# maxim2266/csvplus

Measured on AMD Instinct MI355X. Metric: joined rows/sec (IndexOn build + chained Join, 1e8-row 3-col orders), higher is better.
Workload: dtype u32; 1 GPU; BASELINE configs[3]: orders(1e8 x {cust_id,prod_id,qty}).Join(UniqueIndexOn customers.id 1e7).Join(UniqueIndexOn products.prod_id 1e5); rows=100000000, customers=10000000, products=100000, rows_this_rank=100000000, exchange=none (1 GPU), output=sorted positions

## Files before the change

csvplus_amd/csrc/chain.hip:

```cpp
#include <type_traits>

#include "probe_device.hpp"

namespace cph {

constexpr int kChainThreads = 256;
constexpr int kChainWaves   = kChainThreads / kWave;
constexpr int kChainRows    = 8;
constexpr int kWaveTile     = kWave * kChainRows;
constexpr int kChainTile    = kChainThreads * kChainRows;
constexpr int kChainMasks   = kChainRows * kChainWaves;
constexpr int kMaxChain     = 4;

struct ChainStepArg {
    DevCol col;
    const uint8_t* codec;
    const uint32_t* rowtab;
    const uint2* ranktab;
    int32_t positions;
    int32_t ranktab_lds;
    const uint4* hash;
    uint32_t hash_sectors;
    uint32_t hash_slice_mask;
    int32_t src;
// ... 340 lines not shown
        uint32_t wave_matches = 0;
        const uint64_t mword = (tile * kChainWaves + wave) * kChainRows;
#pragma unroll
        for (int k = 0; k < kChainRows; k++) {
            const bool ok = (okm >> k) & 1u;
            const uint64_t bal = __ballot(ok);
            wave_matches += (uint32_t)__popcll(bal);
            if (lane == 0) masks[mword + k] = bal;
            if (ok) {
#pragma unroll
                for (int s = 0; s < S; s++) (a.out_rows[s] + wr.rbase)[wr.rel[k]] = brow[s][k];
            }
        }
        if (lane == 0) wave_counts[tile * kChainWaves + wave] = wave_matches;
    }
}

__global__ __launch_bounds__(256) void k_sum_counts(const uint32_t* __restrict__ counts, uint64_t n,
                                                   unsigned long long* __restrict__ total) {
    __shared__ uint64_t s_w[256 / kWave];
    uint64_t t = 0;
    const uint64_t stride = (uint64_t)gridDim.x * 256;
    for (uint64_t i = (uint64_t)blockIdx.x * 256 + threadIdx.x; i < n; i += stride) t += counts[i];
    t = wave_sum(t);
    if (lane_id() == 0) s_w[wave_id()] = t;
    __syncthreads();
    if (threadIdx.x == 0) {
        uint64_t r = 0;
        for (int w = 0; w < 256 / kWave; w++) r += s_w[w];
        if (r) atomicAdd(total, (unsigned long long)r);
    }
}

__global__ __launch_bounds__(256) void k_sum_counts_report(const uint32_t* __restrict__ counts, uint64_t n, unsigned long long* __restrict__ acc,
                                                          uint32_t* __restrict__ ticket, unsigned long long* __restrict__ host_out) {
    __shared__ uint64_t s_w[256 / kWave];
    uint64_t t = 0;
    const uint64_t stride = (uint64_t)gridDim.x * 256;
    for (uint64_t i = (uint64_t)blockIdx.x * 256 + threadIdx.x; i < n; i += stride) t += counts[i];
    t = wave_sum(t);
    if (lane_id() == 0) s_w[wave_id()] = t;
    __syncthreads();
    if (threadIdx.x == 0) {
        uint64_t r = 0;
        for (int w = 0; w < 256 / kWave; w++) r += s_w[w];
        if (r) atomicAdd(acc, (unsigned long long)r);
        __threadfence();
        if (atomicAdd(ticket, 1u) == gridDim.x - 1u) {
            const unsigned long long total = atomicExch(acc, 0ull);
            atomicExch(ticket, 0u);
            *host_out = total;
            __threadfence_system();
        }
    }
}

template <int S>
__global__ __launch_bounds__(kChainThreads) void k_chain_compact(ChainArgs dense_rows, uint64_t probe_base,
                                                                const uint64_t* __restrict__ masks,
                                                                const uint32_t* __restrict__ wave_base, uint64_t ntiles,
                                                                uint64_t* __restrict__ out_stream, ChainArgs out_rows) {
    const int lane = lane_id(), wave = wave_id();
    const uint64_t lt = lanemask_lt();
    for (uint64_t tile = blockIdx.x; tile < ntiles; tile += gridDim.x) {
        const uint64_t wt = tile * kChainWaves + wave;
        uint64_t pos = wave_base[wt];
#pragma unroll
        for (int k = 0; k < kChainRows; k++) {
            const uint64_t m = masks[wt * kChainRows + k];
            if ((m >> lane) & 1ull) {
                const uint64_t row = wt * kWaveTile + (uint64_t)k * kWave + lane;
                const uint64_t p = pos + (uint64_t)__popcll(m & lt);
                out_stream[p] = probe_base + row;
#pragma unroll
                for (int s = 0; s < S; s++) out_rows.out_rows[s][p] = dense_rows.out_rows[s][row];
            }
            pos += (uint64_t)__popcll(m);
        }
    }
}

__global__ void k_compose_u64(const uint64_t* __restrict__ src, const uint64_t* __restrict__ idx, uint64_t* __restrict__ dst,
                              uint64_t n) {
    const uint64_t stride = (uint64_t)gridDim.x * blockDim.x;
// ... 261 lines not shown
         {&k_chain_dense<S, false, true, false>, &k_chain_dense<S, false, true, true>}},
        {{&k_chain_dense<S, true, false, false>, &k_chain_dense<S, true, false, true>},
         {&k_chain_dense<S, true, true, false>, &k_chain_dense<S, true, true, true>}}};
    KernelFn kernel = variants[long_keys ? 1 : 0][wide ? 1 : 0][(dbg && !dep) ? 1 : 0];
    if (!dbg && ctx->chain_rows4 != 0 && ((S == 2 && long_keys && wide) || (S >= 3 && (long_keys || wide)) || S == 4 || ctx->chain_rows4 == 2)) {
        static const KernelFn r4[2][2] = {{&k_chain_dense<S, false, false, false, 0u, 4>, &k_chain_dense<S, false, true, false, 0u, 4>},
                                          {&k_chain_dense<S, true, false, false, 0u, 4>, &k_chain_dense<S, true, true, false, 0u, 4>}};
        kernel = r4[long_keys ? 1 : 0][wide ? 1 : 0];
    }
    if constexpr (S >= 2) {
        if (dep) kernel = &k_chain_dense<S, true, true, false, 0u, 4, true>;
    }
    if (lean) {
        constexpr uint32_t kAll = (1u << S) - 1u;
        if (lean == kAll) kernel = &k_chain_dense<S, false, false, false, kAll>;
        if constexpr (S == 2) {
            if (lean == 1u) kernel = &k_chain_dense<S, false, false, false, 1u>;
            if (lean == 2u) kernel = &k_chain_dense<S, false, false, false, 2u>;
        }
    }
    int per_cu = 1, cus = 256;
    CPH_TRY(kernel_setup(ctx, reinterpret_cast<const void*>(kernel), kChainThreads, lds, &per_cu));
    CPH_TRY(device_cus(ctx, &cus));
    const unsigned grid = (unsigned)std::min<uint64_t>(ntiles, (uint64_t)cus * (uint64_t)per_cu);
    {
        ProfScope ps(ctx, prof_name, 0);
        hipLaunchKernelGGL(kernel, dim3(grid), dim3(kChainThreads), lds, ctx->stream, args, nprobe, probe_base,
                           ntiles, d_masks, d_counts, dep ? 0 : dbg, largs);
    }
    if (host_total) {
        DevBuf& acc = ctx->self_clean[ctx->stream_slot].sum;
        CPH_TRY(self_clean_block(ctx, &acc, 16));
        ProfScope ps(ctx, "k_sum_counts", 4.0 * (double)ncounts);
        const unsigned sgrid = (unsigned)std::min<uint64_t>((ncounts + 255) / 256, 512);
        hipLaunchKernelGGL(k_sum_counts_report, dim3(sgrid), dim3(256), 0, ctx->stream, d_counts, ncounts, acc.as<unsigned long long>(),
                           acc.as<uint32_t>() + 2, reinterpret_cast<unsigned long long*>(host_total));
    } else if (d_total) {
        ProfScope ps(ctx, "k_sum_counts", 4.0 * (double)ncounts);
        CPH_HIP_TRY(hipMemsetAsync(d_total, 0, sizeof(uint64_t), ctx->stream));
        const unsigned sgrid = (unsigned)std::min<uint64_t>((ncounts + 255) / 256, 512);
        hipLaunchKernelGGL(k_sum_counts, dim3(sgrid), dim3(256), 0, ctx->stream, d_counts, ncounts,
                           reinterpret_cast<unsigned long long*>(d_total));
    }
    CPH_HIP_TRY(hipGetLastError());
    if (args_out) *args_out = args;
    if (grid_out) *grid_out = grid;
    return {};
}

bool chain_fast_path_ok(const ChainStep* steps, int nsteps);

Status chain_enqueue_dense(cph_ctx* ctx, const ChainStep* steps, int nsteps, uint64_t nprobe, uint64_t probe_base,
                           uint32_t* const* d_rows, uint64_t* d_masks, uint32_t* d_counts, uint64_t* d_total, bool positions) {
    switch (nsteps) {
    case 1: return enqueue_dense<1>(ctx, steps, nprobe, probe_base, d_rows, d_masks, d_counts, d_total, nullptr, nullptr, positions);
    case 2: return enqueue_dense<2>(ctx, steps, nprobe, probe_base, d_rows, d_masks, d_counts, d_total, nullptr, nullptr, positions);
    case 3: return enqueue_dense<3>(ctx, steps, nprobe, probe_base, d_rows, d_masks, d_counts, d_total, nullptr, nullptr, positions);
    case 4: return enqueue_dense<4>(ctx, steps, nprobe, probe_base, d_rows, d_masks, d_counts, d_total, nullptr, nullptr, positions);
    }
    return {CPH_ERR_INVALID, "bad chain length"};
}
template <int S>
static Status enqueue_codes(cph_ctx* ctx, const cph_index* const* idx, const uint32_t* const* d_codes, uint64_t nprobe, uint32_t* const* d_rows,
                            uint64_t* d_masks, uint32_t* d_counts, uint64_t* d_total, bool positions) {
    const uint64_t ntiles = (nprobe + kChainTile - 1) / kChainTile;
    CodeArgs args{};
    for (int s = 0; s < S; s++) {
        const cph_index* ix = idx[s];
        if (ix->nkeycols < 1 || ix->codec.nwords != 1 || !ix->codec.key32 || !ix->windows.empty() || ix->first_dup != UINT64_MAX)
// ... 83 lines not shown
    for (int s = 0; s < S; s++) {
        if (steps[s].source == 0) {
            ind[ni] = steps[s];
            irows[ni++] = rows[s];
            continue;
        }
        const int t = (steps[s].source < 0 ? -steps[s].source : steps[s].source) - 1;
        const int j = pa.n++;
        dep_of[s] = j;
        pa.src_dep[j] = dep_of[t];
        pa.src_rows[j] = rows[t];
        pa.tab[j] = tabs[s].as<uint32_t>();
        pa.out_rows[j] = rows[s];
    }
    switch (ni) {
    case 1: CPH_TRY(enqueue_dense<1>(ctx, ind, nprobe, probe_base, irows, masks, counts, nullptr, nullptr, grid_out, positions)); break;
    case 2: CPH_TRY(enqueue_dense<2>(ctx, ind, nprobe, probe_base, irows, masks, counts, nullptr, nullptr, grid_out, positions)); break;
    case 3: CPH_TRY(enqueue_dense<3>(ctx, ind, nprobe, probe_base, irows, masks, counts, nullptr, nullptr, grid_out, positions)); break;
    default: return {CPH_ERR_INVALID, "a chain needs a step keyed by the stream"};
    }
    {
        int per_cu = 1, cus = 256;
        CPH_TRY(kernel_setup(ctx, reinterpret_cast<const void*>(&k_chain_prejoined), kChainThreads, 0, &per_cu));
        CPH_TRY(device_cus(ctx, &cus));
        const unsigned grid = (unsigned)std::min<uint64_t>(ntiles, (uint64_t)cus * (uint64_t)per_cu);
        ProfScope ps(ctx, "k_chain_prejoined", (double)nprobe * 8.0 * pa.n);
        hipLaunchKernelGGL(k_chain_prejoined, dim3(grid), dim3(kChainThreads), 0, ctx->stream, pa, nprobe, ntiles, masks, counts);
        CPH_HIP_TRY(hipGetLastError());
    }
    {
        DevBuf& acc = ctx->self_clean[ctx->stream_slot].sum;
        CPH_TRY(self_clean_block(ctx, &acc, 16));
        ProfScope ps(ctx, "k_sum_counts", 4.0 * (double)ncounts);
        const unsigned sgrid = (unsigned)std::min<uint64_t>((ncounts + 255) / 256, 512);
        hipLaunchKernelGGL(k_sum_counts_report, dim3(sgrid), dim3(256), 0, ctx->stream, counts, ncounts, acc.as<unsigned long long>(),
                           acc.as<uint32_t>() + 2, reinterpret_cast<unsigned long long*>(host_total));
        CPH_HIP_TRY(hipGetLastError());
    }
    return {};
}

template <int S>
static Status run_fast(cph_ctx* ctx, const ChainStep* steps, uint64_t nprobe, uint64_t probe_base, ChainOut* out, bool positions) {
    const uint64_t ntiles = (nprobe + kChainTile - 1) / kChainTile;
    const uint64_t ncounts = ntiles * kChainWaves;
    uint32_t* rows[kMaxChain] = {nullptr};
    for (int s = 0; s < S; s++) {
        CPH_TRY(out->build_row[s].alloc(&ctx->pool, nprobe * sizeof(uint32_t)));
        rows[s] = out->build_row[s].as<uint32_t>();
    }
    DevBuf masks, counts;
    CPH_TRY(masks.alloc(&ctx->pool, ntiles * kChainMasks * sizeof(uint64_t)));
    CPH_TRY(counts.alloc(&ctx->pool, ncounts * sizeof(uint32_t)));
    volatile uint64_t* h = reinterpret_cast<volatile uint64_t*>(host_word(ctx, 2));
    if (!h) return {CPH_ERR_HIP, "no pinned host memory for the match total"};
    ChainArgs args{};
    unsigned grid = 1;
    bool prejoin = ctx->chain_prejoin != 0;
    {
        bool dep = false;
        for (int s = 0; s < S; s++) {
            if (steps[s].source == 0) continue;
            dep = true;
            const int t = (steps[s].source < 0 ? -steps[s].source : steps[s].source) - 1;
            if (steps[t].index->nrows * 2 > nprobe) prejoin = false;
        }
        prejoin = prejoin && dep;
    }
    if (prejoin) {
// ... 30 lines not shown
    for (int s = 0; s < S; s++) out->build_row[s] = std::move(fin.build_row[s]);
    return {};
}

static Status prejoin_general_step(cph_ctx* ctx, const ChainStep* steps, int s, int t, const uint32_t* h, const uint32_t* h_perm, uint64_t n_in, bool positions,
                                   DevBuf* cur_stream, DevBuf* cur_rows, uint64_t* n_out, bool* all) {
    const uint64_t nt = steps[s].cols[0].nrows;
    ChainStep one = steps[s];
    one.source = 0;
    DevBuf tab, tmask, tcount;
    CPH_TRY(tab.alloc(&ctx->pool, nt * sizeof(uint32_t)));
    CPH_TRY(tmask.alloc(&ctx->pool, chain_dense_mask_words(nt) * sizeof(uint64_t)));
    CPH_TRY(tcount.alloc(&ctx->pool, chain_dense_count_words(nt) * sizeof(uint32_t)));
    CPH_HIP_TRY(hipMemsetAsync(tab.get(), 0xFF, nt * sizeof(uint32_t), ctx->stream));
    uint32_t* r1[kMaxChain] = {tab.as<uint32_t>(), nullptr, nullptr, nullptr};
    CPH_TRY(enqueue_dense<1>(ctx, &one, nt, 0, r1, tmask.as<uint64_t>(), tcount.as<uint32_t>(), nullptr, nullptr, nullptr, positions, nullptr,
                             "k_chain_prejoin_table"));
    const uint64_t ntiles = (n_in + kPjTile - 1) / kPjTile;
    DevBuf v, counts;
    CPH_TRY(v.alloc(&ctx->pool, n_in * sizeof(uint32_t)));
    CPH_TRY(counts.alloc(&ctx->pool, (ntiles + 1) * sizeof(uint32_t)));
    volatile uint64_t* host_total = reinterpret_cast<volatile uint64_t*>(host_word(ctx, 2));
    if (!host_total) return {CPH_ERR_HIP, "no pinned host memory for the match total"};
    {
        ProfScope ps(ctx, "k_prejoin_tuples", (double)n_in * (h_perm ? 16.0 : 12.0));
        hipLaunchKernelGGL(k_prejoin_tuples, dim3((unsigned)ntiles), dim3(kPjThreads), 0, ctx->stream, tab.as<uint32_t>(), h, h_perm, n_in, v.as<uint32_t>(),
                           counts.as<uint32_t>());
        CPH_HIP_TRY(hipGetLastError());
    }
    {
        DevBuf& acc = ctx->self_clean[ctx->stream_slot].sum;
        CPH_TRY(self_clean_block(ctx, &acc, 16));
        ProfScope ps(ctx, "k_sum_counts", 4.0 * (double)ntiles);
        const unsigned sgrid = (unsigned)std::min<uint64_t>((ntiles + 255) / 256, 512);
        hipLaunchKernelGGL(k_sum_counts_report, dim3(sgrid), dim3(256), 0, ctx->stream, counts.as<uint32_t>(), ntiles, acc.as<unsigned long long>(),
                           acc.as<uint32_t>() + 2, reinterpret_cast<unsigned long long*>(const_cast<uint64_t*>(host_total)));
        CPH_HIP_TRY(hipGetLastError());
    }
    CPH_HIP_TRY(hipStreamSynchronize(ctx->stream));
    const uint64_t m = host_total[0];
    *all = m == n_in;
    *n_out = m;
    if (m == n_in) {
        cur_rows[s] = std::move(v);
        return {};
    }
    if (m == 0) return {};
    CPH_TRY(exclusive_scan_u32(ctx, counts.as<uint32_t>(), ntiles));
    PjCompactArgs ca{};
    DevBuf nstream, nrows[CPH_MAX_CHAIN];
    CPH_TRY(nstream.alloc(&ctx->pool, m * sizeof(uint64_t)));
    ca.src64 = cur_stream->as<uint64_t>();
    ca.dst64 = nstream.as<uint64_t>();
    for (int u = 0; u < s; u++) {
        CPH_TRY(nrows[u].alloc(&ctx->pool, m * sizeof(uint32_t)));
        ca.src32[ca.n32] = cur_rows[u].as<uint32_t>();
        ca.dst32[ca.n32++] = nrows[u].as<uint32_t>();
    }
    CPH_TRY(nrows[s].alloc(&ctx->pool, m * sizeof(uint32_t)));
    ca.src32[ca.n32] = v.as<uint32_t>();
    ca.dst32[ca.n32++] = nrows[s].as<uint32_t>();
    {
        ProfScope ps(ctx, "k_compose", (double)n_in * (12.0 + 4.0 * s) + (double)m * (12.0 + 4.0 * s));
        hipLaunchKernelGGL(k_prejoin_compact, dim3((unsigned)ntiles), dim3(kPjThreads), 0, ctx->stream, ca, v.as<uint32_t>(), n_in, counts.as<uint32_t>());
        CPH_HIP_TRY(hipGetLastError());
    }
    *cur_stream = std::move(nstream);
    for (int u = 0; u <= s; u++) cur_rows[u] = std::move(nrows[u]);
    return {};
// ... 101 lines not shown
```

csvplus_amd/csrc/keycodec.hip:

```cpp
#include <algorithm>
#include <cmath>
#include <mutex>

#include "codec_device.hpp"
#include "host_encode_kernels.hpp"

namespace cph {

constexpr int kStatsThreads = 256;
constexpr int kStatsRows = 8;

template <class B, bool SEG>
__global__ __launch_bounds__(kStatsThreads) void k_col_stats(DevCol col, uint32_t* __restrict__ g_minmax,
                                                            uint32_t* __restrict__ g_mask) {
    __shared__ __attribute__((aligned(16))) uint8_t s_flag[kMaxKeyBytes * 256];
    __shared__ uint32_t s_min, s_max;
    {
        uint4* z = reinterpret_cast<uint4*>(s_flag);
        for (int i = threadIdx.x; i < kMaxKeyBytes * 256 / 16; i += kStatsThreads) z[i] = make_uint4(0, 0, 0, 0);
    }
    if (threadIdx.x == 0) { s_min = 0xFFFFFFFFu; s_max = 0; }
    __syncthreads();

    uint32_t mn = 0xFFFFFFFFu, mx = 0;
// ... 1015 lines not shown
                const bool ok = hit[k] && v[k].len <= vmax && plen[k] <= (uint32_t)kWideBytes && slen[k] <= smaxlen;
                if (!ok && base + (uint64_t)k * kSplitThreads + threadIdx.x < tile_end) missed = 1;
                acc[k] = (OUT)(hit[k] ? e[k] - 1 : 0u) * pmult;
                v[k].window(plen[k], &w0[k], &w1[k]);
            }
            for (uint32_t q = 0; q < smaxlen; q++) {
                const CPH_LDS OUT* lp = s_lutw + q * (uint32_t)kLutStride;
#pragma unroll
                for (int k = 0; k < kSplitRows; k++) {
                    const uint64_t src = q < 8u ? w0[k] : w1[k];
                    const uint32_t sym = q < slen[k] ? ((uint32_t)(src >> (8u * (q & 7u))) & 0xFFu) + 1u : 0u;
                    acc[k] += lp[sym];
                }
            }
#pragma unroll
            for (int k = 0; k < kSplitRows; k++) {
                const uint64_t i = base + (uint64_t)k * kSplitThreads + threadIdx.x;
                if (i < tile_end) {
                    if (inv && acc[k] >= inv) missed = 1;
                    out[i] = acc[k];
                    if (counts) atomicAdd(&s_hist[(uint32_t)acc[k] & digit_mask], 1u);
                }
            }
        }
        if (counts) {
            lds_atomics_barrier();
            for (uint32_t x = threadIdx.x; x < bins; x += kSplitThreads) counts[(uint64_t)x * ntiles + tile] = s_hist[x];
            __syncthreads();
        }
    }
    if (__ballot(missed) && lane_id() == 0) *miss = 1u;
}

__global__ __launch_bounds__(kSplitThreads) void k_sample_fixed8(DevCol col, uint64_t step, uint64_t n, SplitSample* __restrict__ out,
                                                                SplitSample* __restrict__ host_out) {
    __shared__ uint32_t s_mask[8 * 8];
    __shared__ uint32_t s_last;
    const uint32_t W = col.fixed_width;
    if (threadIdx.x < 64) s_mask[threadIdx.x] = 0;
    __syncthreads();
    const uint64_t stride = (uint64_t)gridDim.x * kSplitThreads;
    for (uint64_t i = (uint64_t)blockIdx.x * kSplitThreads + threadIdx.x; i < n; i += stride) {
        uint64_t b, l;
        value_span_whole(col, i * step, &b, &l);
        ValueRegs<1> v;
        v.load(col, b, l);
        for (uint32_t q = 0; q < W; q++) {
            const uint32_t byte = (uint32_t)(v.c[0] >> (8u * q)) & 0xFFu, bit = 1u << (byte & 31u);
            uint32_t* w = &s_mask[q * 8u + (byte >> 5)];
            if (!(*(volatile uint32_t*)w & bit)) atomicOr(w, bit);
        }
    }
    lds_atomics_barrier();
    if (threadIdx.x < 64) {
        const uint32_t bits = s_mask[threadIdx.x];
        uint32_t* gm = &out->mask[0][0] + threadIdx.x;
        if (bits && (__hip_atomic_load(gm, __ATOMIC_RELAXED, __HIP_MEMORY_SCOPE_AGENT) & bits) != bits) atomicOr(gm, bits);
    }
    uint32_t* ticket = reinterpret_cast<uint32_t*>(out + 1);
    __threadfence();
    __syncthreads();
    if (threadIdx.x == 0) s_last = atomicAdd(ticket, 1u) == gridDim.x - 1u ? 1u : 0u;
    __syncthreads();
    if (s_last) {
        uint32_t* src = &out->mask[0][0];
        uint32_t* dst = &host_out->mask[0][0];
        for (uint32_t i = threadIdx.x; i < (uint32_t)(kSplitMaxValue * 8); i += kSplitThreads) dst[i] = i < 64u ? atomicExch(&src[i], 0u) : 0u;
        if (threadIdx.x == 0) {
            host_out->maxlen = W;
            host_out->minlen_inv = ~W;
            atomicExch(ticket, 0u);
        }
        __threadfence_system();
    }
}

int codec_virtual_cols(const CodecHost& cd, const DevCol* real, int nreal, DevCol* out) {
    int nv = 0;
    for (int c = 0; c < nreal; c++) {
        if (cd.has_split() && c == cd.split_col) {
            DevCol a = real[c], b = real[c];
            a.split = b.split = (uint16_t)(0x100u | cd.split_byte);
            a.part = 0;
            b.part = 1;
            out[nv++] = a;
            out[nv++] = b;
        } else {
            out[nv++] = real[c];
        }
    }
    return nv;
}

bool codec_wide_perfect_hash(CodecHost* codec) {
    CodecHost& cd = *codec;
    const size_t n = cd.wdict.size();
    cd.wide_disp.clear();
    cd.wide_slots.clear();
    if (n == 0 || n > (size_t)kWideDictMax) return false;
    std::vector<uint32_t> h(n);
// ... 142 lines not shown
        for (int sym = 0; sym < kLutStride; sym++) trial.lut[((size_t)p0 + i) * kLutStride + (size_t)sym] = 0;
    }
    trial.split_col = c;
    trial.split_byte = (uint8_t)d;
    trial.split_maxlen = (int32_t)st.vmax;
    trial.wdict = std::move(dict);
    if (!codec_wide_perfect_hash(&trial)) return {};
    CPH_TRY(codec_split_words(&trial));
    if (ctx->codec_debug)
        fprintf(stderr, "codec_try_split: column %d cut at 0x%02x: %zu prefixes (<= %u bytes), suffix %u..%u bytes: %d word(s), %d bits, sort cost %.0f (plain: %.1f bits%s)\n",
                c, d, trial.wdict.size(), st.pmax, smin, st.smax, trial.nwords, trial.word_bits[0], codec_sort_cost(trial), plain_bits,
                stats ? "" : " by the sample");
    *out = std::move(trial);
    *usable = true;
    return {};
}

bool codec_sample_applies(const cph_ctx* ctx, const DevCol* cols, int32_t ncols, uint64_t n) {
    return ctx->stats_sample != 0 && ncols == 1 && cols[0].fixed_width >= 1 && cols[0].fixed_width <= (uint32_t)kSplitMaxValue &&
           !cols[0].segmented() && n >= (1ull << 20);
}
size_t codec_sample_bytes() { return sizeof(SplitSample); }
Status codec_sample_launch(cph_ctx* ctx, const DevCol& col, uint64_t n, const void** host_copy) {
    const uint64_t step = n >> 16;
    const uint64_t nsel = (n + step - 1) / step;
    DevBuf& acc = ctx->self_clean[ctx->stream_slot].sample;
    CPH_TRY(self_clean_block(ctx, &acc, sizeof(SplitSample) + 16));
    uint32_t* hw = host_word(ctx, (uint32_t)(sizeof(SplitSample) / 4));
    if (!hw) return {CPH_ERR_HIP, "no pinned host memory for the sample's statistics"};
    ProfScope ps(ctx, "k_split_count", 0);
    uint64_t nblk = (nsel + kSplitThreads - 1) / kSplitThreads;
    if (nblk > 1024) nblk = 1024;
    if (col.fixed_width <= 8)
        hipLaunchKernelGGL(k_sample_fixed8, dim3((unsigned)nblk), dim3(kSplitThreads), 0, ctx->stream, col, step, nsel, acc.as<SplitSample>(),
                           reinterpret_cast<SplitSample*>(hw));
    else
        hipLaunchKernelGGL(k_split_count, dim3((unsigned)nblk), dim3(kSplitThreads), 0, ctx->stream, col, step, nsel, acc.as<SplitSample>(),
                           reinterpret_cast<SplitSample*>(hw));
    if (hipGetLastError() != hipSuccess) {
        acc.reset();
        return {CPH_ERR_HIP, "k_split_count launch failed"};
    }
    *host_copy = hw;
    return {};
}
void codec_sample_finish(const DevCol& col, const void* host_copy, std::vector<ColStats>* out) {
    const SplitSample* sm = static_cast<const SplitSample*>(host_copy);
    out->assign(1, ColStats{});
    ColStats& st = (*out)[0];
    st.minlen = st.maxlen = col.fixed_width;
    static_assert(sizeof(sm->mask) <= sizeof(st.mask), "the sample's positions must fit ColStats");
    memcpy(st.mask, sm->mask, sizeof sm->mask);
}
bool codec_sample_checked(const CodecHost& cd, const DevCol* cols) {
    return !cd.has_split() && !cd.has_groups() && cd.ncols == 1 && cd.nwords == 1 && codec_premultiplied_bits(cd) != 0 && !cols[0].segmented();
}

Status codec_try_split(cph_ctx* ctx, const DevCol* cols, int32_t ncols, uint64_t n, const std::vector<ColStats>* stats, CodecHost* codec,
                       bool speculate, bool* speculated) {
    if (speculated) *speculated = false;
    if (!ctx->codec_split || n < (1ull << 16) || ncols >= kMaxKeyCols) return {};
    if (stats && (codec->key32 || codec->has_groups())) return {};
    if (!stats && ncols != 1) return {};
    int c = -1;
    double most = 0, plain_bits = 0;
    if (stats) {
        for (int k = 0; k < ncols; k++) {
// ... 943 lines not shown
```

csvplus_amd/csrc/window_sort.hip:

```cpp
#include "cph_internal.hpp"
#include "codec_device.hpp"
#include "device_utils.hpp"

namespace cph {

constexpr int kWpThreads = 512;
constexpr int kWpItems = 16;
constexpr int kWpTile = kWpThreads * kWpItems;
constexpr int kWpMaxBuckets = 2048;
constexpr int kWinBits = 14;
constexpr uint32_t kWinSlots = 1u << kWinBits;
constexpr uint32_t kWinEmpty = 0xFFFFFFFFu;
constexpr int kPlaceThreads = 512;

struct WpArgs {
    const uint64_t* keys;
    ArithPlan ap;
    const uint32_t* codes;
    const uint64_t* entries;
    const uint32_t* src_count;
    uint64_t n;
    uint32_t src_cap;
    uint32_t tiles_per_src;
    uint32_t shift;
    uint32_t nb;
    uint64_t* dst;
    uint32_t* dst_count;
    uint32_t states;
    uint32_t row_base;
    uint32_t* flag;
};

template <int SRC>
__global__ __launch_bounds__(kWpThreads) void k_win_partition(WpArgs a) {
    constexpr bool FROM_CODES = SRC != 0;
    extern __shared__ __attribute__((aligned(16))) uint8_t smem[];
    __shared__ uint32_t s_tmp[kWpThreads / kWave + 1];
    const uint32_t nbp = (a.nb + (uint32_t)kWpThreads - 1u) & ~((uint32_t)kWpThreads - 1u);
    uint64_t* s_ent = reinterpret_cast<uint64_t*>(smem);
    uint32_t* s_hist = reinterpret_cast<uint32_t*>(s_ent + kWpTile);
    uint32_t* s_start = s_hist + nbp;
    uint32_t* s_delta = s_start + nbp;
    const uint32_t sb = blockIdx.x / a.tiles_per_src, tl = blockIdx.x % a.tiles_per_src;
    uint64_t cnt = a.n;
    if constexpr (!FROM_CODES) {
        const uint32_t c = a.src_count[sb];
        cnt = c < a.src_cap ? c : a.src_cap;
    }
    const uint64_t t0 = (uint64_t)tl * kWpTile;
    if (t0 >= cnt) return;
    const uint32_t m = cnt - t0 < (uint64_t)kWpTile ? (uint32_t)(cnt - t0) : (uint32_t)kWpTile;
    const uint64_t src0 = FROM_CODES ? t0 : (uint64_t)sb * a.src_cap + t0;
    const uint32_t t = threadIdx.x;
    for (uint32_t i = t; i < nbp; i += kWpThreads) s_hist[i] = 0;
    __syncthreads();
    typedef unsigned int u32x4 __attribute__((ext_vector_type(4)));
    uint32_t code[kWpItems], row[kWpItems], rank[kWpItems];
    if constexpr (SRC == 2) {
        uint64_t c0[kWpItems];
        uint32_t okm = 0;
#pragma unroll
        for (int j = 0; j < kWpItems / 4; j++) {
            const uint32_t i4 = 4u * ((uint32_t)j * kWpThreads + t);
            if (i4 + 3 < m) {
                const u32x4 v0 = reinterpret_cast<const u32x4*>(a.keys + src0 + i4)[0], v1 = reinterpret_cast<const u32x4*>(a.keys + src0 + i4)[1];
                c0[4 * j] = (uint64_t)v0.x | ((uint64_t)v0.y << 32);
                c0[4 * j + 1] = (uint64_t)v0.z | ((uint64_t)v0.w << 32);
                c0[4 * j + 2] = (uint64_t)v1.x | ((uint64_t)v1.y << 32);
                c0[4 * j + 3] = (uint64_t)v1.z | ((uint64_t)v1.w << 32);
                okm |= 0xFu << (4 * j);
            } else {
#pragma unroll
                for (int c = 0; c < 4; c++) {
                    c0[4 * j + c] = i4 + c < m ? a.keys[src0 + i4 + c] : 0ull;
                    okm |= (i4 + c < m ? 1u : 0u) << (4 * j + c);
                }
            }
#pragma unroll
            for (int c = 0; c < 4; c++) row[4 * j + c] = a.row_base + (uint32_t)(t0 + i4 + c);
        }
        const uint32_t have = okm;
        encode_rows_arith<kWpItems, uint32_t>(a.ap, c0, code, &okm);
        bool bad = false;
#pragma unroll
        for (int k = 0; k < kWpItems; k++) {
            const bool ok = ((okm >> k) & 1u) && code[k] < a.states;
            bad |= ((have >> k) & 1u) && !ok;
            code[k] = ok ? code[k] : kWinEmpty;
        }
        if (__ballot(bad) && lane_id() == 0) *a.flag = 1u;
    } else if constexpr (SRC == 1) {
        const bool vec = m == (uint32_t)kWpTile && (((uintptr_t)(a.codes + src0)) & 15) == 0;
#pragma unroll
        for (int j = 0; j < kWpItems / 4; j++) {
            const uint32_t i4 = 4u * ((uint32_t)j * kWpThreads + t);
            uint32_t w[4];
            if (vec) {
                const u32x4 v = reinterpret_cast<const u32x4*>(a.codes + src0)[i4 >> 2];
                w[0] = v.x; w[1] = v.y; w[2] = v.z; w[3] = v.w;
            } else {
#pragma unroll
                for (int c = 0; c < 4; c++) w[c] = i4 + c < m ? a.codes[src0 + i4 + c] : kWinEmpty;
            }
#pragma unroll
            for (int c = 0; c < 4; c++) {
                const bool ok = i4 + c < m && w[c] < a.states;
                code[4 * j + c] = ok ? w[c] : kWinEmpty;
                row[4 * j + c] = a.row_base + (uint32_t)(t0 + i4 + c);
            }
        }
    } else {
        const bool vec = m == (uint32_t)kWpTile;
#pragma unroll
        for (int j = 0; j < kWpItems / 2; j++) {
            const uint32_t i2 = 2u * ((uint32_t)j * kWpThreads + t);
            if (vec) {
                const u32x4 v = reinterpret_cast<const u32x4*>(a.entries + src0)[i2 >> 1];
                row[2 * j] = v.x; code[2 * j] = v.y; row[2 * j + 1] = v.z; code[2 * j + 1] = v.w;
            } else {
#pragma unroll
                for (int c = 0; c < 2; c++) {
                    const uint64_t e = i2 + c < m ? a.entries[src0 + i2 + c] : ~0ull;
                    row[2 * j + c] = (uint32_t)e;
                    code[2 * j + c] = i2 + c < m ? (uint32_t)(e >> 32) : kWinEmpty;
                }
            }
        }
    }
#pragma unroll
    for (int k = 0; k < kWpItems; k++) rank[k] = code[k] != kWinEmpty ? atomicAdd(&s_hist[code[k] >> a.shift], 1u) : 0u;
    lds_atomics_barrier();
    uint32_t tot;
    {
        const uint32_t per = nbp / kWpThreads;
        uint32_t h[kWpMaxBuckets / kWpThreads], sum = 0;
#pragma unroll
        for (int k = 0; k < kWpMaxBuckets / kWpThreads; k++) {
            h[k] = (uint32_t)k < per ? s_hist[t * per + k] : 0u;
            sum += h[k];
        }
        uint32_t run = block_exclusive_sum<uint32_t, kWpThreads>(sum, s_tmp, &tot);
#pragma unroll
        for (int k = 0; k < kWpMaxBuckets / kWpThreads; k++) {
            if ((uint32_t)k < per) {
                const uint32_t b = t * per + k;
                s_start[b] = run;
                if (h[k]) s_delta[b] = atomicAdd(&a.dst_count[(uint64_t)sb * a.nb + b], h[k]) - run;
                run += h[k];
            }
        }
    }
    __syncthreads();
#pragma unroll
    for (int k = 0; k < kWpItems; k++)
        if (code[k] != kWinEmpty) s_ent[s_start[code[k] >> a.shift] + rank[k]] = ((uint64_t)code[k] << 32) | row[k];
    __syncthreads();
    const uint32_t cap = 1u << a.shift, mask = cap - 1u;
    bool over = false;
    uint64_t e[kWpItems];
    uint32_t pos[kWpItems];
#pragma unroll
    for (int k = 0; k < kWpItems; k++) {
        const uint32_t i = (uint32_t)k * kWpThreads + t;
        e[k] = s_ent[i < tot ? i : 0u];
    }
#pragma unroll
    for (int k = 0; k < kWpItems; k++) {
        const uint32_t i = (uint32_t)k * kWpThreads + t;
        pos[k] = s_delta[i < tot ? (uint32_t)(e[k] >> 32) >> a.shift : 0u] + i;
    }
#pragma unroll
    for (int k = 0; k < kWpItems; k++) {
        const uint32_t i = (uint32_t)k * kWpThreads + t;
        if (i < tot) {
            const uint32_t w = (uint32_t)(e[k] >> 32), b = w >> a.shift;
            if (pos[k] < cap) a.dst[(((uint64_t)sb * a.nb + b) << a.shift) + pos[k]] = ((uint64_t)(w & mask) << 32) | (uint32_t)e[k];
            else over = true;
        }
    }
    if (__ballot(over) && lane_id() == 0) *a.flag = 1u;
}

__global__ __launch_bounds__(1024) void k_win_offsets(const uint32_t* __restrict__ counts, uint32_t nwin, uint32_t* __restrict__ off) {
    __shared__ uint32_t s_tmp[1024 / kWave + 1];
    uint32_t carry = 0;
    for (uint32_t base = 0; base < nwin; base += 1024) {
        const uint32_t i = base + threadIdx.x;
        uint32_t v = i < nwin ? counts[i] : 0u;
        v = v < kWinSlots ? v : kWinSlots;
        uint32_t total;
        const uint32_t ex = block_exclusive_sum<uint32_t, 1024>(v, s_tmp, &total);
        if (i < nwin) off[i] = carry + ex;
        carry += total;
    }
}

__global__ __launch_bounds__(kPlaceThreads) void k_win_place(const uint64_t* __restrict__ entries, uint32_t* __restrict__ counts,
                                                            const uint32_t* __restrict__ off, uint64_t n, uint32_t* __restrict__ perm,
                                                            uint32_t* __restrict__ sorted, uint32_t* __restrict__ flag,
                                                            uint32_t* __restrict__ clear_also, uint32_t nclear, uint2* __restrict__ ranktab,
                                                            uint32_t rank_blocks) {
    extern __shared__ __attribute__((aligned(16))) uint8_t smem[];
    __shared__ uint32_t s_wcount[kPlaceThreads / kWave];
    typedef unsigned int u32x4 __attribute__((ext_vector_type(4)));
    uint32_t* win = reinterpret_cast<uint32_t*>(smem);
    const uint32_t g = blockIdx.x, t = threadIdx.x;
// ... 52 lines not shown
    }
}

Status WindowSort::begin(cph_ctx* ctx, uint64_t n_, uint64_t states_) {
    n = n_;
    states = states_;
    const uint64_t nwin = (states + kWinSlots - 1) >> kWinBits;
    two = nwin > (uint64_t)kWpMaxBuckets;
    int k2 = 0;
    if (two) {
        int wb = 0;
        while ((1ull << wb) < nwin) wb++;
        k2 = (wb + 1) / 2;
    }
    nb2 = 1u << k2;
    shift1 = (uint32_t)kWinBits + (uint32_t)k2;
    nb1 = two ? (states + (1ull << shift1) - 1) >> shift1 : nwin;
    if (nb1 > (uint64_t)kWpMaxBuckets) return {CPH_ERR_INVALID, "direct_sort_windows: code space too large"};
    nwin_total = two ? nb1 * nb2 : nwin;
    CPH_TRY(ent1.alloc(&ctx->pool, (nb1 << shift1) * sizeof(uint64_t)));
    if (two) CPH_TRY(ent2.alloc(&ctx->pool, (nwin_total << kWinBits) * sizeof(uint64_t)));
    const uint64_t nwords = nb1 + (two ? nwin_total : 0);
    words = &ctx->self_clean[ctx->stream_slot].win;
    CPH_TRY(self_clean_block(ctx, words, nwords * sizeof(uint32_t)));
    cur1 = words->as<uint32_t>();
    cur2 = two ? cur1 + nb1 : cur1;
    started = true;
    return {};
}
WindowSort::~WindowSort() {
    if (started && !finished && words) words->reset();
}

static size_t win_partition_lds(uint32_t nb) {
    const uint32_t nbp = (nb + (uint32_t)kWpThreads - 1u) & ~((uint32_t)kWpThreads - 1u);
    return (size_t)kWpTile * 8 + (size_t)nbp * 12;
}

Status WindowSort::add(cph_ctx* ctx, const uint32_t* codes, uint64_t row0, uint64_t m, uint32_t* flag, const uint64_t* keys, const ArithPlan* ap) {
    if (m == 0) return {};
    WpArgs a{};
    a.codes = codes;
    a.keys = keys;
    if (keys) a.ap = *ap;
    a.n = m;
    a.tiles_per_src = (uint32_t)((m + kWpTile - 1) / kWpTile);
    a.shift = shift1;
    a.nb = (uint32_t)nb1;
    a.dst = ent1.as<uint64_t>();
    a.dst_count = cur1;
    a.states = (uint32_t)states;
    a.row_base = (uint32_t)row0;
    a.flag = flag;
    const size_t lds = win_partition_lds(a.nb);
    if (keys) {
        CPH_TRY(kernel_setup(ctx, reinterpret_cast<const void*>(&k_win_partition<2>), kWpThreads, lds, nullptr));
        ProfScope ps(ctx, "k_win_partition", 16.0 * (double)m);
        hipLaunchKernelGGL(k_win_partition<2>, dim3(a.tiles_per_src), dim3(kWpThreads), lds, ctx->stream, a);
    } else {
        CPH_TRY(kernel_setup(ctx, reinterpret_cast<const void*>(&k_win_partition<1>), kWpThreads, lds, nullptr));
        ProfScope ps(ctx, "k_win_partition", 12.0 * (double)m);
        hipLaunchKernelGGL(k_win_partition<1>, dim3(a.tiles_per_src), dim3(kWpThreads), lds, ctx->stream, a);
    }
    CPH_HIP_TRY(hipGetLastError());
    return {};
}

Status WindowSort::finish(cph_ctx* ctx, uint32_t* perm_out, uint32_t* sorted_out, uint32_t* flag, void* ranktab, uint64_t rank_blocks) {
    const bool need_off = states != n;
    DevBuf offsets;
    if (need_off) CPH_TRY(offsets.alloc(&ctx->pool, nwin_total * sizeof(uint32_t)));
    uint32_t* off = offsets.as<uint32_t>();
    if (two) {
        WpArgs a{};
        a.entries = ent1.as<uint64_t>();
        a.src_count = cur1;
        a.src_cap = 1u << shift1;
        a.tiles_per_src = (a.src_cap + kWpTile - 1) / kWpTile;
        a.shift = (uint32_t)kWinBits;
        a.nb = nb2;
        a.dst = ent2.as<uint64_t>();
        a.dst_count = cur2;
        a.flag = flag;
        const size_t lds = win_partition_lds(a.nb);
        CPH_TRY(kernel_setup(ctx, reinterpret_cast<const void*>(&k_win_partition<0>), kWpThreads, lds, nullptr));
        ProfScope ps(ctx, "k_win_partition", 16.0 * (double)n);
        hipLaunchKernelGGL(k_win_partition<0>, dim3((unsigned)(nb1 * a.tiles_per_src)), dim3(kWpThreads), lds, ctx->stream, a);
        CPH_HIP_TRY(hipGetLastError());
    }
    uint32_t* counts = two ? cur2 : cur1;
    if (need_off) {
        ProfScope ps(ctx, "k_win_place", 0);
        hipLaunchKernelGGL(k_win_offsets, dim3(1), dim3(1024), 0, ctx->stream, counts, (uint32_t)nwin_total, off);
    }
    {
        const size_t lds = (size_t)kWinSlots * sizeof(uint32_t);
        CPH_TRY(kernel_setup(ctx, reinterpret_cast<const void*>(&k_win_place), kPlaceThreads, lds, nullptr));
        ProfScope ps(ctx, "k_win_place", 16.0 * (double)n);
        hipLaunchKernelGGL(k_win_place, dim3((unsigned)nwin_total), dim3(kPlaceThreads), lds, ctx->stream, two ? ent2.as<uint64_t>() : ent1.as<uint64_t>(),
                           counts, need_off ? off : nullptr, n, perm_out, sorted_out, flag, cur1, two ? (uint32_t)nb1 : 0u,
                           static_cast<uint2*>(ranktab), (uint32_t)rank_blocks);
    }
    CPH_HIP_TRY(hipGetLastError());
    finished = true;
    return {};
}

Status direct_sort_windows(cph_ctx* ctx, const uint32_t* codes, uint64_t n, uint64_t states, uint32_t* perm_out, uint32_t* sorted_out,
                           uint32_t* flag, void* ranktab, uint64_t rank_blocks) {
    if (n == 0) return {};
    WindowSort ws;
    CPH_TRY(ws.begin(ctx, n, states));
    CPH_TRY(ws.add(ctx, codes, 0, n, flag));
    return ws.finish(ctx, perm_out, sorted_out, flag, ranktab, rank_blocks);
}
Status direct_sort_windows_keys(cph_ctx* ctx, const uint64_t* keys, const ArithPlan& ap, uint64_t n, uint64_t states, uint32_t* perm_out,
                                uint32_t* sorted_out, uint32_t* flag, void* ranktab, uint64_t rank_blocks) {
    if (n == 0) return {};
    WindowSort ws;
    CPH_TRY(ws.begin(ctx, n, states));
// ... 14 lines not shown
```

Baseline: 133.0 billion rows/s.

## Vectorize count summation, batch sampling loads, and widen one-level window partition blocks

The final count-sum kernel now reads counts as uint4 with several loads in flight and a capped grid. It folds the completion ticket into the high bits of the accumulator atomic, which removes a separate ticket atomic and fence. The fixed-width sampler batches eight row loads per thread and caps its grid, with a leaner release/acquire handoff to the last block. Single-level window partitioning uses 1024-thread blocks with 8 items each, keeping the same tile size. These are small launch- and latency-bound tweaks to minor kernels, and the packed ticket limits the sum to 56 bits.

```diff
diff --git a/csvplus_amd/csrc/chain.hip b/csvplus_amd/csrc/chain.hip
--- a/csvplus_amd/csrc/chain.hip
+++ b/csvplus_amd/csrc/chain.hip
@@ -396,24 +396,41 @@
     }
 }
 
+constexpr int kSumBlocks = 32;
+constexpr int kSumLoads = 8;
+constexpr int kSumTicketShift = 56;
+static unsigned sum_counts_grid(uint64_t n) {
+    const uint64_t per_block = 256ull * 4 * kSumLoads;
+    return (unsigned)std::max<uint64_t>(1, std::min<uint64_t>((n + per_block - 1) / per_block, (uint64_t)kSumBlocks));
+}
 __global__ __launch_bounds__(256) void k_sum_counts_report(const uint32_t* __restrict__ counts, uint64_t n, unsigned long long* __restrict__ acc,
-                                                          uint32_t* __restrict__ ticket, unsigned long long* __restrict__ host_out) {
+                                                          unsigned long long* __restrict__ host_out) {
     __shared__ uint64_t s_w[256 / kWave];
     uint64_t t = 0;
-    const uint64_t stride = (uint64_t)gridDim.x * 256;
-    for (uint64_t i = (uint64_t)blockIdx.x * 256 + threadIdx.x; i < n; i += stride) t += counts[i];
+    const uint64_t stride = (uint64_t)gridDim.x * 256, gt = (uint64_t)blockIdx.x * 256 + threadIdx.x;
+    const uint64_t nv = ((uintptr_t)counts & 15) == 0 ? n >> 2 : 0;
+    const uint4* __restrict__ c4 = reinterpret_cast<const uint4*>(counts);
+    for (uint64_t v0 = gt; v0 < nv; v0 += stride * kSumLoads) {
+        uint4 x[kSumLoads];
+#pragma unroll
+        for (int k = 0; k < kSumLoads; k++) {
+            const uint64_t v = v0 + (uint64_t)k * stride;
+            x[k] = v < nv ? c4[v] : make_uint4(0, 0, 0, 0);
+        }
+#pragma unroll
+        for (int k = 0; k < kSumLoads; k++) t += (uint64_t)x[k].x + x[k].y + x[k].z + x[k].w;
+    }
+    for (uint64_t i = nv * 4 + gt; i < n; i += stride) t += counts[i];
     t = wave_sum(t);
     if (lane_id() == 0) s_w[wave_id()] = t;
     __syncthreads();
     if (threadIdx.x == 0) {
         uint64_t r = 0;
         for (int w = 0; w < 256 / kWave; w++) r += s_w[w];
-        if (r) atomicAdd(acc, (unsigned long long)r);
-        __threadfence();
-        if (atomicAdd(ticket, 1u) == gridDim.x - 1u) {
-            const unsigned long long total = atomicExch(acc, 0ull);
-            atomicExch(ticket, 0u);
-            *host_out = total;
+        const unsigned long long before = atomicAdd(acc, (unsigned long long)r + (1ull << kSumTicketShift));
+        if ((before >> kSumTicketShift) == gridDim.x - 1u) {
+            atomicExch(acc, 0ull);
+            *host_out = (before & ((1ull << kSumTicketShift) - 1ull)) + r;
             __threadfence_system();
         }
     }
@@ -741,9 +758,9 @@
         DevBuf& acc = ctx->self_clean[ctx->stream_slot].sum;
         CPH_TRY(self_clean_block(ctx, &acc, 16));
         ProfScope ps(ctx, "k_sum_counts", 4.0 * (double)ncounts);
-        const unsigned sgrid = (unsigned)std::min<uint64_t>((ncounts + 255) / 256, 512);
+        const unsigned sgrid = sum_counts_grid(ncounts);
         hipLaunchKernelGGL(k_sum_counts_report, dim3(sgrid), dim3(256), 0, ctx->stream, d_counts, ncounts, acc.as<unsigned long long>(),
-                           acc.as<uint32_t>() + 2, reinterpret_cast<unsigned long long*>(host_total));
+                           reinterpret_cast<unsigned long long*>(host_total));
     } else if (d_total) {
         ProfScope ps(ctx, "k_sum_counts", 4.0 * (double)ncounts);
         CPH_HIP_TRY(hipMemsetAsync(d_total, 0, sizeof(uint64_t), ctx->stream));
@@ -893,9 +910,9 @@
         DevBuf& acc = ctx->self_clean[ctx->stream_slot].sum;
         CPH_TRY(self_clean_block(ctx, &acc, 16));
         ProfScope ps(ctx, "k_sum_counts", 4.0 * (double)ncounts);
-        const unsigned sgrid = (unsigned)std::min<uint64_t>((ncounts + 255) / 256, 512);
+        const unsigned sgrid = sum_counts_grid(ncounts);
         hipLaunchKernelGGL(k_sum_counts_report, dim3(sgrid), dim3(256), 0, ctx->stream, counts, ncounts, acc.as<unsigned long long>(),
-                           acc.as<uint32_t>() + 2, reinterpret_cast<unsigned long long*>(host_total));
+                           reinterpret_cast<unsigned long long*>(host_total));
         CPH_HIP_TRY(hipGetLastError());
     }
     return {};
@@ -992,9 +1009,9 @@
         DevBuf& acc = ctx->self_clean[ctx->stream_slot].sum;
         CPH_TRY(self_clean_block(ctx, &acc, 16));
         ProfScope ps(ctx, "k_sum_counts", 4.0 * (double)ntiles);
-        const unsigned sgrid = (unsigned)std::min<uint64_t>((ntiles + 255) / 256, 512);
+        const unsigned sgrid = sum_counts_grid(ntiles);
         hipLaunchKernelGGL(k_sum_counts_report, dim3(sgrid), dim3(256), 0, ctx->stream, counts.as<uint32_t>(), ntiles, acc.as<unsigned long long>(),
-                           acc.as<uint32_t>() + 2, reinterpret_cast<unsigned long long*>(const_cast<uint64_t*>(host_total)));
+                           reinterpret_cast<unsigned long long*>(const_cast<uint64_t*>(host_total)));
         CPH_HIP_TRY(hipGetLastError());
     }
     CPH_HIP_TRY(hipStreamSynchronize(ctx->stream));
diff --git a/csvplus_amd/csrc/keycodec.hip b/csvplus_amd/csrc/keycodec.hip
--- a/csvplus_amd/csrc/keycodec.hip
+++ b/csvplus_amd/csrc/keycodec.hip
@@ -1071,6 +1071,8 @@
     if (__ballot(missed) && lane_id() == 0) *miss = 1u;
 }
 
+constexpr int kFixed8Rows = 8;
+constexpr int kFixed8Blocks = 64;
 __global__ __launch_bounds__(kSplitThreads) void k_sample_fixed8(DevCol col, uint64_t step, uint64_t n, SplitSample* __restrict__ out,
                                                                 SplitSample* __restrict__ host_out) {
     __shared__ uint32_t s_mask[8 * 8];
@@ -1079,32 +1081,43 @@
     if (threadIdx.x < 64) s_mask[threadIdx.x] = 0;
     __syncthreads();
     const uint64_t stride = (uint64_t)gridDim.x * kSplitThreads;
-    for (uint64_t i = (uint64_t)blockIdx.x * kSplitThreads + threadIdx.x; i < n; i += stride) {
-        uint64_t b, l;
-        value_span_whole(col, i * step, &b, &l);
-        ValueRegs<1> v;
-        v.load(col, b, l);
+    for (uint64_t i0 = (uint64_t)blockIdx.x * kSplitThreads + threadIdx.x; i0 < n; i0 += stride * kFixed8Rows) {
+        uint64_t c[kFixed8Rows];
+#pragma unroll
+        for (int k = 0; k < kFixed8Rows; k++) {
+            const uint64_t i = i0 + (uint64_t)k * stride;
+            ValueRegs<1> v;
+            v.load(col, (i < n ? i : i0) * step * W, W);
+            c[k] = v.c[0];
+        }
         for (uint32_t q = 0; q < W; q++) {
-            const uint32_t byte = (uint32_t)(v.c[0] >> (8u * q)) & 0xFFu, bit = 1u << (byte & 31u);
-            uint32_t* w = &s_mask[q * 8u + (byte >> 5)];
-            if (!(*(volatile uint32_t*)w & bit)) atomicOr(w, bit);
+            uint32_t seen[kFixed8Rows];
+#pragma unroll
+            for (int k = 0; k < kFixed8Rows; k++) {
+                const uint32_t byte = (uint32_t)(c[k] >> (8u * q)) & 0xFFu;
+                seen[k] = *(volatile CPH_LDS uint32_t*)&s_mask[q * 8u + (byte >> 5)];
+            }
+#pragma unroll
+            for (int k = 0; k < kFixed8Rows; k++) {
+                const uint32_t byte = (uint32_t)(c[k] >> (8u * q)) & 0xFFu, bit = 1u << (byte & 31u);
+                if (!(seen[k] & bit)) atomicOr(&s_mask[q * 8u + (byte >> 5)], bit);
+            }
         }
     }
     lds_atomics_barrier();
+    uint32_t* ticket = reinterpret_cast<uint32_t*>(out + 1);
     if (threadIdx.x < 64) {
         const uint32_t bits = s_mask[threadIdx.x];
         uint32_t* gm = &out->mask[0][0] + threadIdx.x;
         if (bits && (__hip_atomic_load(gm, __ATOMIC_RELAXED, __HIP_MEMORY_SCOPE_AGENT) & bits) != bits) atomicOr(gm, bits);
-    }
-    uint32_t* ticket = reinterpret_cast<uint32_t*>(out + 1);
-    __threadfence();
+        __builtin_amdgcn_fence(__ATOMIC_RELEASE, "agent");
+        asm volatile("s_waitcnt vmcnt(0)" ::: "memory");
+        if (threadIdx.x == 0) s_last = atomicAdd(ticket, 1u) == gridDim.x - 1u ? 1u : 0u;
+    }
     __syncthreads();
-    if (threadIdx.x == 0) s_last = atomicAdd(ticket, 1u) == gridDim.x - 1u ? 1u : 0u;
-    __syncthreads();
-    if (s_last) {
-        uint32_t* src = &out->mask[0][0];
-        uint32_t* dst = &host_out->mask[0][0];
-        for (uint32_t i = threadIdx.x; i < (uint32_t)(kSplitMaxValue * 8); i += kSplitThreads) dst[i] = i < 64u ? atomicExch(&src[i], 0u) : 0u;
+    if (s_last && threadIdx.x < 64) {
+        __builtin_amdgcn_fence(__ATOMIC_ACQUIRE, "agent");
+        (&host_out->mask[0][0])[threadIdx.x] = atomicExch(&out->mask[0][0] + threadIdx.x, 0u);
         if (threadIdx.x == 0) {
             host_out->maxlen = W;
             host_out->minlen_inv = ~W;
@@ -1313,7 +1326,7 @@
     uint64_t nblk = (nsel + kSplitThreads - 1) / kSplitThreads;
     if (nblk > 1024) nblk = 1024;
     if (col.fixed_width <= 8)
-        hipLaunchKernelGGL(k_sample_fixed8, dim3((unsigned)nblk), dim3(kSplitThreads), 0, ctx->stream, col, step, nsel, acc.as<SplitSample>(),
+        hipLaunchKernelGGL(k_sample_fixed8, dim3((unsigned)std::min<uint64_t>(nblk, (uint64_t)kFixed8Blocks)), dim3(kSplitThreads), 0, ctx->stream, col, step, nsel, acc.as<SplitSample>(),
                            reinterpret_cast<SplitSample*>(hw));
     else
         hipLaunchKernelGGL(k_split_count, dim3((unsigned)nblk), dim3(kSplitThreads), 0, ctx->stream, col, step, nsel, acc.as<SplitSample>(),
diff --git a/csvplus_amd/csrc/window_sort.hip b/csvplus_amd/csrc/window_sort.hip
--- a/csvplus_amd/csrc/window_sort.hip
+++ b/csvplus_amd/csrc/window_sort.hip
@@ -6,7 +6,10 @@
 
 constexpr int kWpThreads = 512;
 constexpr int kWpItems = 16;
+constexpr int kWpThreadsOneLevel = 1024;
+constexpr int kWpItemsOneLevel = 8;
 constexpr int kWpTile = kWpThreads * kWpItems;
+static_assert(kWpThreadsOneLevel * kWpItemsOneLevel == kWpTile, "one tile size");
 constexpr int kWpMaxBuckets = 2048;
 constexpr int kWinBits = 14;
 constexpr uint32_t kWinSlots = 1u << kWinBits;
@@ -31,14 +34,15 @@
     uint32_t* flag;
 };
 
-template <int SRC>
-__global__ __launch_bounds__(kWpThreads) void k_win_partition(WpArgs a) {
+template <int SRC, int THREADS, int ITEMS>
+__global__ __launch_bounds__(THREADS) void k_win_partition(WpArgs a) {
     constexpr bool FROM_CODES = SRC != 0;
+    constexpr int TILE = THREADS * ITEMS;
     extern __shared__ __attribute__((aligned(16))) uint8_t smem[];
-    __shared__ uint32_t s_tmp[kWpThreads / kWave + 1];
-    const uint32_t nbp = (a.nb + (uint32_t)kWpThreads - 1u) & ~((uint32_t)kWpThreads - 1u);
+    __shared__ uint32_t s_tmp[THREADS / kWave + 1];
+    const uint32_t nbp = (a.nb + (uint32_t)THREADS - 1u) & ~((uint32_t)THREADS - 1u);
     uint64_t* s_ent = reinterpret_cast<uint64_t*>(smem);
-    uint32_t* s_hist = reinterpret_cast<uint32_t*>(s_ent + kWpTile);
+    uint32_t* s_hist = reinterpret_cast<uint32_t*>(s_ent + TILE);
     uint32_t* s_start = s_hist + nbp;
     uint32_t* s_delta = s_start + nbp;
     const uint32_t sb = blockIdx.x / a.tiles_per_src, tl = blockIdx.x % a.tiles_per_src;
@@ -47,21 +51,21 @@
         const uint32_t c = a.src_count[sb];
         cnt = c < a.src_cap ? c : a.src_cap;
     }
-    const uint64_t t0 = (uint64_t)tl * kWpTile;
+    const uint64_t t0 = (uint64_t)tl * TILE;
     if (t0 >= cnt) return;
-    const uint32_t m = cnt - t0 < (uint64_t)kWpTile ? (uint32_t)(cnt - t0) : (uint32_t)kWpTile;
+    const uint32_t m = cnt - t0 < (uint64_t)TILE ? (uint32_t)(cnt - t0) : (uint32_t)TILE;
     const uint64_t src0 = FROM_CODES ? t0 : (uint64_t)sb * a.src_cap + t0;
     const uint32_t t = threadIdx.x;
-    for (uint32_t i = t; i < nbp; i += kWpThreads) s_hist[i] = 0;
+    for (uint32_t i = t; i < nbp; i += THREADS) s_hist[i] = 0;
     __syncthreads();
     typedef unsigned int u32x4 __attribute__((ext_vector_type(4)));
-    uint32_t code[kWpItems], row[kWpItems], rank[kWpItems];
+    uint32_t code[ITEMS], row[ITEMS], rank[ITEMS];
     if constexpr (SRC == 2) {
-        uint64_t c0[kWpItems];
+        uint64_t c0[ITEMS];
         uint32_t okm = 0;
 #pragma unroll
-        for (int j = 0; j < kWpItems / 4; j++) {
-            const uint32_t i4 = 4u * ((uint32_t)j * kWpThreads + t);
+        for (int j = 0; j < ITEMS / 4; j++) {
+            const uint32_t i4 = 4u * ((uint32_t)j * THREADS + t);
             if (i4 + 3 < m) {
                 const u32x4 v0 = reinterpret_cast<const u32x4*>(a.keys + src0 + i4)[0], v1 = reinterpret_cast<const u32x4*>(a.keys + src0 + i4)[1];
                 c0[4 * j] = (uint64_t)v0.x | ((uint64_t)v0.y << 32);
@@ -80,20 +84,20 @@
             for (int c = 0; c < 4; c++) row[4 * j + c] = a.row_base + (uint32_t)(t0 + i4 + c);
         }
         const uint32_t have = okm;
-        encode_rows_arith<kWpItems, uint32_t>(a.ap, c0, code, &okm);
+        encode_rows_arith<ITEMS, uint32_t>(a.ap, c0, code, &okm);
         bool bad = false;
 #pragma unroll
-        for (int k = 0; k < kWpItems; k++) {
+        for (int k = 0; k < ITEMS; k++) {
             const bool ok = ((okm >> k) & 1u) && code[k] < a.states;
             bad |= ((have >> k) & 1u) && !ok;
             code[k] = ok ? code[k] : kWinEmpty;
         }
         if (__ballot(bad) && lane_id() == 0) *a.flag = 1u;
     } else if constexpr (SRC == 1) {
-        const bool vec = m == (uint32_t)kWpTile && (((uintptr_t)(a.codes + src0)) & 15) == 0;
-#pragma unroll
-        for (int j = 0; j < kWpItems / 4; j++) {
-            const uint32_t i4 = 4u * ((uint32_t)j * kWpThreads + t);
+        const bool vec = m == (uint32_t)TILE && (((uintptr_t)(a.codes + src0)) & 15) == 0;
+#pragma unroll
+        for (int j = 0; j < ITEMS / 4; j++) {
+            const uint32_t i4 = 4u * ((uint32_t)j * THREADS + t);
             uint32_t w[4];
             if (vec) {
                 const u32x4 v = reinterpret_cast<const u32x4*>(a.codes + src0)[i4 >> 2];
@@ -110,10 +114,10 @@
             }
         }
     } else {
-        const bool vec = m == (uint32_t)kWpTile;
-#pragma unroll
-        for (int j = 0; j < kWpItems / 2; j++) {
-            const uint32_t i2 = 2u * ((uint32_t)j * kWpThreads + t);
+        const bool vec = m == (uint32_t)TILE;
+#pragma unroll
+        for (int j = 0; j < ITEMS / 2; j++) {
+            const uint32_t i2 = 2u * ((uint32_t)j * THREADS + t);
             if (vec) {
                 const u32x4 v = reinterpret_cast<const u32x4*>(a.entries + src0)[i2 >> 1];
                 row[2 * j] = v.x; code[2 * j] = v.y; row[2 * j + 1] = v.z; code[2 * j + 1] = v.w;
@@ -128,20 +132,20 @@
         }
     }
 #pragma unroll
-    for (int k = 0; k < kWpItems; k++) rank[k] = code[k] != kWinEmpty ? atomicAdd(&s_hist[code[k] >> a.shift], 1u) : 0u;
+    for (int k = 0; k < ITEMS; k++) rank[k] = code[k] != kWinEmpty ? atomicAdd(&s_hist[code[k] >> a.shift], 1u) : 0u;
     lds_atomics_barrier();
     uint32_t tot;
     {
-        const uint32_t per = nbp / kWpThreads;
-        uint32_t h[kWpMaxBuckets / kWpThreads], sum = 0;
-#pragma unroll
-        for (int k = 0; k < kWpMaxBuckets / kWpThreads; k++) {
+        const uint32_t per = nbp / THREADS;
+        uint32_t h[kWpMaxBuckets / THREADS], sum = 0;
+#pragma unroll
+        for (int k = 0; k < kWpMaxBuckets / THREADS; k++) {
             h[k] = (uint32_t)k < per ? s_hist[t * per + k] : 0u;
             sum += h[k];
         }
-        uint32_t run = block_exclusive_sum<uint32_t, kWpThreads>(sum, s_tmp, &tot);
-#pragma unroll
-        for (int k = 0; k < kWpMaxBuckets / kWpThreads; k++) {
+        uint32_t run = block_exclusive_sum<uint32_t, THREADS>(sum, s_tmp, &tot);
+#pragma unroll
+        for (int k = 0; k < kWpMaxBuckets / THREADS; k++) {
             if ((uint32_t)k < per) {
                 const uint32_t b = t * per + k;
                 s_start[b] = run;
@@ -152,26 +156,26 @@
     }
     __syncthreads();
 #pragma unroll
-    for (int k = 0; k < kWpItems; k++)
+    for (int k = 0; k < ITEMS; k++)
         if (code[k] != kWinEmpty) s_ent[s_start[code[k] >> a.shift] + rank[k]] = ((uint64_t)code[k] << 32) | row[k];
     __syncthreads();
     const uint32_t cap = 1u << a.shift, mask = cap - 1u;
     bool over = false;
-    uint64_t e[kWpItems];
-    uint32_t pos[kWpItems];
-#pragma unroll
-    for (int k = 0; k < kWpItems; k++) {
-        const uint32_t i = (uint32_t)k * kWpThreads + t;
+    uint64_t e[ITEMS];
+    uint32_t pos[ITEMS];
+#pragma unroll
+    for (int k = 0; k < ITEMS; k++) {
+        const uint32_t i = (uint32_t)k * THREADS + t;
         e[k] = s_ent[i < tot ? i : 0u];
     }
 #pragma unroll
-    for (int k = 0; k < kWpItems; k++) {
-        const uint32_t i = (uint32_t)k * kWpThreads + t;
+    for (int k = 0; k < ITEMS; k++) {
+        const uint32_t i = (uint32_t)k * THREADS + t;
         pos[k] = s_delta[i < tot ? (uint32_t)(e[k] >> 32) >> a.shift : 0u] + i;
     }
 #pragma unroll
-    for (int k = 0; k < kWpItems; k++) {
-        const uint32_t i = (uint32_t)k * kWpThreads + t;
+    for (int k = 0; k < ITEMS; k++) {
+        const uint32_t i = (uint32_t)k * THREADS + t;
         if (i < tot) {
             const uint32_t w = (uint32_t)(e[k] >> 32), b = w >> a.shift;
             if (pos[k] < cap) a.dst[(((uint64_t)sb * a.nb + b) << a.shift) + pos[k]] = ((uint64_t)(w & mask) << 32) | (uint32_t)e[k];
@@ -290,9 +294,14 @@
     if (started && !finished && words) words->reset();
 }
 
-static size_t win_partition_lds(uint32_t nb) {
-    const uint32_t nbp = (nb + (uint32_t)kWpThreads - 1u) & ~((uint32_t)kWpThreads - 1u);
-    return (size_t)kWpTile * 8 + (size_t)nbp * 12;
+template <int SRC, int THREADS, int ITEMS>
+static Status win_partition_launch(cph_ctx* ctx, const WpArgs& a, unsigned grid, double bytes) {
+    const uint32_t nbp = (a.nb + (uint32_t)THREADS - 1u) & ~((uint32_t)THREADS - 1u);
+    const size_t lds = (size_t)THREADS * ITEMS * 8 + (size_t)nbp * 12;
+    CPH_TRY(kernel_setup(ctx, reinterpret_cast<const void*>(&k_win_partition<SRC, THREADS, ITEMS>), THREADS, lds, nullptr));
+    ProfScope ps(ctx, "k_win_partition", bytes);
+    hipLaunchKernelGGL((k_win_partition<SRC, THREADS, ITEMS>), dim3(grid), dim3(THREADS), lds, ctx->stream, a);
+    return {};
 }
 
 Status WindowSort::add(cph_ctx* ctx, const uint32_t* codes, uint64_t row0, uint64_t m, uint32_t* flag, const uint64_t* keys, const ArithPlan* ap) {
@@ -310,15 +319,12 @@
     a.states = (uint32_t)states;
     a.row_base = (uint32_t)row0;
     a.flag = flag;
-    const size_t lds = win_partition_lds(a.nb);
     if (keys) {
-        CPH_TRY(kernel_setup(ctx, reinterpret_cast<const void*>(&k_win_partition<2>), kWpThreads, lds, nullptr));
-        ProfScope ps(ctx, "k_win_partition", 16.0 * (double)m);
-        hipLaunchKernelGGL(k_win_partition<2>, dim3(a.tiles_per_src), dim3(kWpThreads), lds, ctx->stream, a);
+        if (two) CPH_TRY((win_partition_launch<2, kWpThreads, kWpItems>(ctx, a, a.tiles_per_src, 16.0 * (double)m)));
+        else CPH_TRY((win_partition_launch<2, kWpThreadsOneLevel, kWpItemsOneLevel>(ctx, a, a.tiles_per_src, 16.0 * (double)m)));
     } else {
-        CPH_TRY(kernel_setup(ctx, reinterpret_cast<const void*>(&k_win_partition<1>), kWpThreads, lds, nullptr));
-        ProfScope ps(ctx, "k_win_partition", 12.0 * (double)m);
-        hipLaunchKernelGGL(k_win_partition<1>, dim3(a.tiles_per_src), dim3(kWpThreads), lds, ctx->stream, a);
+        if (two) CPH_TRY((win_partition_launch<1, kWpThreads, kWpItems>(ctx, a, a.tiles_per_src, 12.0 * (double)m)));
+        else CPH_TRY((win_partition_launch<1, kWpThreadsOneLevel, kWpItemsOneLevel>(ctx, a, a.tiles_per_src, 12.0 * (double)m)));
     }
     CPH_HIP_TRY(hipGetLastError());
     return {};
@@ -340,10 +346,7 @@
         a.dst = ent2.as<uint64_t>();
         a.dst_count = cur2;
         a.flag = flag;
-        const size_t lds = win_partition_lds(a.nb);
-        CPH_TRY(kernel_setup(ctx, reinterpret_cast<const void*>(&k_win_partition<0>), kWpThreads, lds, nullptr));
-        ProfScope ps(ctx, "k_win_partition", 16.0 * (double)n);
-        hipLaunchKernelGGL(k_win_partition<0>, dim3((unsigned)(nb1 * a.tiles_per_src)), dim3(kWpThreads), lds, ctx->stream, a);
+        CPH_TRY((win_partition_launch<0, kWpThreads, kWpItems>(ctx, a, (unsigned)(nb1 * a.tiles_per_src), 16.0 * (double)n)));
         CPH_HIP_TRY(hipGetLastError());
     }
     uint32_t* counts = two ? cur2 : cur1;
```

Result: faster. 139.4 billion rows/s, median of 6 (+4.9%).
